# JuliaQuantumControl/QuOptimalControl.jl

Measured on AMD Instinct MI355X. Metric: GRAPE gradient-evals/sec, higher is better.
Workload: dtype f64; 1 GPU; C3: UnitaryGate 4x4, K=4, N=500 slices, ensemble E=1024 (one GPU, 1024 members/GPU), T=2.0; step = host->host grape_eval; parallelism=single GPU

## Files before the change

### quoptimalcontrol.jl_amd/csrc/cmatp.hpp

```cpp
#pragma once
#include <hip/hip_runtime.h>

#include "cmat.hpp"

namespace grape {

template <int N>
struct PMat {
    static constexpr int NC = N / 2;
    double re[N * (N / 2)];
    double im[N * (N / 2)];
};

GRAPE_DEV double pair_swap(double v)
{
    int lo = __double2loint(v), hi = __double2hiint(v);
    lo = __builtin_amdgcn_update_dpp(0, lo, 0xB1, 0xF, 0xF, true);
    hi = __builtin_amdgcn_update_dpp(0, hi, 0xB1, 0xF, 0xF, true);
    return __hiloint2double(hi, lo);
}

template <int N>
GRAPE_DEV void fetch_partner(PMat<N> &out, const PMat<N> &in)
{
// ... 222 lines not shown
                }
            }
            c.re[r + jl * N] = sr;
            c.im[r + jl * N] = si;
        }
        {
            double d = 0.0;
#pragma unroll
            for (int s = 0; s < N; ++s) {
                d = fma(g.re[s + jl * N], g.re[s + jl * N], d);
                d = fma(g.im[s + jl * N], g.im[s + jl * N], d);
            }
            c.re[jl + jl * N] = -d;
            c.im[jl + jl * N] = 0.0;
        }
#pragma unroll
        for (int rl = 0; rl < jl; ++rl) {
            double sr = 0.0, si = 0.0;
#pragma unroll
            for (int s = 0; s < N; ++s) {
                const double ar = g.re[s + rl * N], ai = -g.im[s + rl * N];
                const double br = g.re[s + jl * N], bi = g.im[s + jl * N];
                sr = fma(ar, br, sr); sr = fma(-ai, bi, sr);
                si = fma(ar, bi, si); si = fma(ai, br, si);
            }
            c.re[rl + jl * N] = -sr;
            c.im[rl + jl * N] = -si;
            c.re[jl + rl * N] = -sr;
            c.im[jl + rl * N] = si;
        }
    }
}

template <int N>
struct PAntiH {
    static constexpr int NC = N / 2;
    double di[NC];
    double ur[NC * NC], ui[NC * NC];
    double ore[NC * NC], oim[NC * NC];
};

template <int N>
GRAPE_DEV void pah_from_mat(PAntiH<N> &h, const PMat<N> &m)
{
    constexpr int NC = N / 2;
#pragma unroll
    for (int jl = 0; jl < NC; ++jl)
#pragma unroll
        for (int rl = 0; rl < NC; ++rl) {
            if (rl == jl)
                h.di[jl] = m.im[jl + jl * N];
            if (rl < jl) {
                h.ur[rl + jl * NC] = m.re[rl + jl * N];
                h.ui[rl + jl * NC] = m.im[rl + jl * N];
            }
            h.ore[rl + jl * NC] = m.re[NC + rl + jl * N];
            h.oim[rl + jl * NC] = m.im[NC + rl + jl * N];
        }
}

template <int N>
GRAPE_DEV void pah_of_scaled(PAntiH<N> &h, const PMat<N> &c, double zr, double zi)
{
    constexpr int NC = N / 2, NE = N * NC;
    PMat<N> Z;
#pragma unroll
    for (int e = 0; e < NE; ++e) {
        Z.re[e] = fma(c.re[e], zr, -c.im[e] * zi);
        Z.im[e] = fma(c.re[e], zi, c.im[e] * zr);
    }
#pragma unroll
    for (int jl = 0; jl < NC; ++jl)
#pragma unroll
        for (int rl = 0; rl < NC; ++rl) {
            if (rl == jl)
                h.di[jl] = Z.im[jl + jl * N];
            if (rl < jl) {
                h.ur[rl + jl * NC] = 0.5 * (Z.re[rl + jl * N] - Z.re[jl + rl * N]);
                h.ui[rl + jl * NC] = 0.5 * (Z.im[rl + jl * N] + Z.im[jl + rl * N]);
            }
            h.ore[rl + jl * NC] = 0.5 * (Z.re[NC + rl + jl * N] - pair_swap(Z.re[NC + jl + rl * N]));
            h.oim[rl + jl * NC] = 0.5 * (Z.im[NC + rl + jl * N] + pair_swap(Z.im[NC + jl + rl * N]));
        }
}

template <int N>
GRAPE_DEV void pah_own(PMat<N> &a, const PAntiH<N> &h)
{
    constexpr int NC = N / 2;
#pragma unroll
    for (int jl = 0; jl < NC; ++jl)
#pragma unroll
        for (int rl = 0; rl < NC; ++rl) {
            if (rl == jl) {
                a.re[rl + jl * N] = 0.0;
                a.im[rl + jl * N] = h.di[jl];
            } else if (rl < jl) {
                a.re[rl + jl * N] = h.ur[rl + jl * NC];
                a.im[rl + jl * N] = h.ui[rl + jl * NC];
            } else {
                a.re[rl + jl * N] = -h.ur[jl + rl * NC];
                a.im[rl + jl * N] = h.ui[jl + rl * NC];
            }
            a.re[NC + rl + jl * N] = h.ore[rl + jl * NC];
            a.im[NC + rl + jl * N] = h.oim[rl + jl * NC];
        }
}

template <int N>
GRAPE_DEV void pah_partner(PMat<N> &par, const PAntiH<N> &h)
{
    constexpr int NC = N / 2;
#pragma unroll
    for (int jl = 0; jl < NC; ++jl)
#pragma unroll
        for (int rl = 0; rl < NC; ++rl) {
            if (rl == jl) {
                par.re[rl + jl * N] = 0.0;
                par.im[rl + jl * N] = pair_swap(h.di[jl]);
            } else if (rl < jl) {
                const double vr = pair_swap(h.ur[rl + jl * NC]), vi = pair_swap(h.ui[rl + jl * NC]);
                par.re[rl + jl * N] = vr;
                par.im[rl + jl * N] = vi;
                par.re[jl + rl * N] = -vr;
                par.im[jl + rl * N] = vi;
            }
            par.re[NC + rl + jl * N] = -h.ore[jl + rl * NC];
            par.im[NC + rl + jl * N] = h.oim[jl + rl * NC];
        }
}

template <int N>
GRAPE_DEV void pmul_antih_a(PMat<N> &c, const PMat<N> &a, const PMat<N> &apar, const PMat<N> &b)
{
    constexpr int NC = N / 2;
#pragma unroll
    for (int jl = 0; jl < NC; ++jl)
#pragma unroll
        for (int r = 0; r < N; ++r) {
            double sr = 0.0, si = 0.0;
#pragma unroll
            for (int kl = 0; kl < NC; ++kl) {
                {
                    const double ar = a.re[r + kl * N], ai = a.im[r + kl * N];
                    const double br = b.re[kl + jl * N], bi = b.im[kl + jl * N];
                    if (r != kl) sr = fma(ar, br, sr);
                    sr = fma(-ai, bi, sr);
                    if (r != kl) si = fma(ar, bi, si);
                    si = fma(ai, br, si);
                }
                {
                    const int rb = flip_block<N>(r);
                    const double ar = apar.re[rb + kl * N], ai = apar.im[rb + kl * N];
                    const double br = b.re[NC + kl + jl * N], bi = b.im[NC + kl + jl * N];
                    if (rb != kl) sr = fma(ar, br, sr);
                    sr = fma(-ai, bi, sr);
                    if (rb != kl) si = fma(ar, bi, si);
                    si = fma(ai, br, si);
                }
            }
            c.re[r + jl * N] = sr;
            c.im[r + jl * N] = si;
        }
}

template <int N>
// ... 104 lines not shown
```

### quoptimalcontrol.jl_amd/csrc/sweep_pair.hip

```cpp
#include "cmatp.hpp"
#include "grape_kernels.hpp"

#ifndef GRAPE_ABL
#define GRAPE_ABL 0
#endif
#ifndef GRAPE_PD
#define GRAPE_PD 2
#endif
#ifndef GRAPE_PLAYOUT
#define GRAPE_PLAYOUT 0
#endif
#ifndef GRAPE_PD_EARLY
#define GRAPE_PD_EARLY 2
#endif
#ifndef GRAPE_PD_EARLY_AT
#define GRAPE_PD_EARLY_AT 0
#endif
#ifndef GRAPE_MBAR
#define GRAPE_MBAR 2
#endif

namespace grape {

enum { PMODE_GENERAL = 0, PMODE_GENERAL_KEEPL = 1, PMODE_UNITARY = 2, PMODE_UNITARY_AH = 3 };
// ... 13 lines not shown
{
#pragma unroll
    for (int jl = 0; jl < N / 2; ++jl)
#pragma unroll
        for (int r = 0; r < N; ++r)
            base[(size_t)gelem<N>(q, r, jl) * stride] = make_double2(m.re[r + jl * N], m.im[r + jl * N]);
}

template <int N>
GRAPE_DEV void pstore_ws_split(double2 *__restrict__ sbase, const unsigned (&voff)[2], size_t stride, const PMat<N> &m)
{
#pragma unroll
    for (int jl = 0; jl < N / 2; ++jl)
#pragma unroll
        for (int r = 0; r < N; ++r) {
            char *row = reinterpret_cast<char *>(sbase + (size_t)((r % (N / 2)) + jl * N) * stride);
            *reinterpret_cast<double2 *>(row + voff[r / (N / 2)]) = make_double2(m.re[r + jl * N], m.im[r + jl * N]);
        }
}

template <int N>
GRAPE_DEV void pload_ws(PMat<N> &m, const double2 *__restrict__ base, size_t stride, int q)
{
#pragma unroll
    for (int jl = 0; jl < N / 2; ++jl)
#pragma unroll
        for (int r = 0; r < N; ++r) {
            const double2 v = base[(size_t)gelem<N>(q, r, jl) * stride];
            m.re[r + jl * N] = v.x;
            m.im[r + jl * N] = v.y;
        }
}

template <int N>
GRAPE_DEV void pload_lds(PMat<N> &m, const double2 *s)
{
#pragma unroll
    for (int e = 0; e < N * (N / 2); ++e) {
        const double2 v = s[e];
        m.re[e] = v.x;
        m.im[e] = v.y;
    }
}

template <int N>
GRAPE_DEV void pstore_lds(double2 *s, const PMat<N> &m)
{
#pragma unroll
    for (int e = 0; e < N * (N / 2); ++e)
        s[e] = make_double2(m.re[e], m.im[e]);
}

GRAPE_DEV void pstamp(unsigned long long *__restrict__ st, int slot)
{
    if (st) {
        const unsigned long long t = __builtin_readcyclecounter();
        if ((threadIdx.x & 63) == 0)
            st[slot] = t;
    }
}

typedef double d2v __attribute__((ext_vector_type(2)));
struct PBuf {
    d2v v[8];
};

GRAPE_DEV void pbuf_issue(PBuf &b, unsigned voff0, unsigned voff1, const double2 *sb0, const double2 *sb1, const double2 *sb4,
                          const double2 *sb5)
{
    asm volatile("global_load_dwordx4 %0, %8, %10\n\t"
                 "global_load_dwordx4 %1, %8, %11\n\t"
                 "global_load_dwordx4 %2, %9, %10\n\t"
                 "global_load_dwordx4 %3, %9, %11\n\t"
                 "global_load_dwordx4 %4, %8, %12\n\t"
                 "global_load_dwordx4 %5, %8, %13\n\t"
                 "global_load_dwordx4 %6, %9, %12\n\t"
                 "global_load_dwordx4 %7, %9, %13"
                 : "=&v"(b.v[0]), "=&v"(b.v[1]), "=&v"(b.v[2]), "=&v"(b.v[3]), "=&v"(b.v[4]), "=&v"(b.v[5]), "=&v"(b.v[6]),
                   "=&v"(b.v[7])
                 : "v"(voff0), "v"(voff1), "s"(sb0), "s"(sb1), "s"(sb4), "s"(sb5)
                 : "memory");
}

template <int YOUNGER>
GRAPE_DEV void pbuf_wait(PBuf &b)
{
    asm volatile("s_waitcnt vmcnt(%8)"
                 : "+v"(b.v[0]), "+v"(b.v[1]), "+v"(b.v[2]), "+v"(b.v[3]), "+v"(b.v[4]), "+v"(b.v[5]), "+v"(b.v[6]), "+v"(b.v[7])
                 : "n"(YOUNGER)
                 : "memory");
}

GRAPE_DEV void pbuf_to_mat(PMat<4> &m, const PBuf &b)
{
#pragma unroll
    for (int e = 0; e < 8; ++e) {
        m.re[e] = b.v[e][0];
        m.im[e] = b.v[e][1];
    }
}

GRAPE_DEV void member_barrier(unsigned *cnt, unsigned target)
{
    asm volatile("s_waitcnt lgkmcnt(0)" ::: "memory");
    if ((threadIdx.x & 63) == 0)
        __hip_atomic_fetch_add(cnt, 1u, __ATOMIC_RELAXED, __HIP_MEMORY_SCOPE_WORKGROUP);
    while (__hip_atomic_load(cnt, __ATOMIC_RELAXED, __HIP_MEMORY_SCOPE_WORKGROUP) < target)
        __builtin_amdgcn_s_sleep(1);
    asm volatile("" ::: "memory");
}

GRAPE_DEV void lds_barrier()
{
    asm volatile("s_waitcnt lgkmcnt(0)" ::: "memory");
    __builtin_amdgcn_s_barrier();
    asm volatile("" ::: "memory");
}

template <int N, int SAND>
GRAPE_DEV double pfigure_of_merit(double zr, double zi)
{
    if (SAND) {
        const double inv = 1.0 / (double)N;
        const double ar = zr * inv, ai = zi * inv;
        return 1.0 - (ar * ar + ai * ai);
    }
    return zr * zr - zi * zi;
}

template <int N, int SAND>
GRAPE_DEV void pwrite_gradient(double *out, const double2 *s_bt, int K, const PMat<N> &M, double zr, double zi,
                               double gs, int p)
{
    constexpr int NE = N * (N / 2);
    PMat<N> Z;
#pragma unroll
    for (int e = 0; e < NE; ++e) {
        if (SAND) {
            Z.re[e] = M.re[e];
            Z.im[e] = M.im[e];
        } else {
            Z.re[e] = fma(M.re[e], zr, -M.im[e] * zi);
            Z.im[e] = fma(M.re[e], zi, M.im[e] * zr);
        }
    }
    double2 b0[NE], b1[NE];
#pragma unroll
    for (int e = 0; e < NE; ++e)
        b0[e] = s_bt[e];
    for (int c = 0; c < K; c += 2) {
        if (c + 1 < K) {
#pragma unroll
            for (int e = 0; e < NE; ++e)
                b1[e] = s_bt[(c + 1) * NE + e];
        }
        double re = 0.0;
#pragma unroll
        for (int e = 0; e < NE; ++e) {
            re = fma(b0[e].x, Z.re[e], re);
            re = fma(-b0[e].y, Z.im[e], re);
        }
        re += pair_swap(re);
        if (p == 0)
            out[c] = gs * re;
        if (c + 1 < K) {
            if (c + 2 < K) {
#pragma unroll
                for (int e = 0; e < NE; ++e)
                    b0[e] = s_bt[(c + 2) * NE + e];
            }
            double r1 = 0.0;
#pragma unroll
            for (int e = 0; e < NE; ++e) {
// ... 279 lines not shown
                    G.re[e] = fma(b0[e].x, x0, G.re[e]);
                    G.im[e] = fma(b0[e].y, x0, G.im[e]);
                }
            }
#pragma unroll
            for (int e = 0; e < NE; ++e)
                b0[e] = sB[c2 * NE + e];
#pragma unroll
            for (int e = 0; e < NE; ++e) {
                G.re[e] = fma(b1[e].x, x1, G.re[e]);
                G.im[e] = fma(b1[e].y, x1, G.im[e]);
            }
        }
        if (p.variant == 0) {
#pragma unroll
            for (int e = 0; e < NE; ++e) {
                const double2 a = sA[e];
                G.re[e] += a.x;
                G.im[e] += a.y;
            }
        }
        return nb;
    };
    auto slice = [&](int j, PMat<N> &G, double nb, const PMat<N> &Qin, PMat<N> &Qout, bool first) {
        PMat<N> P, Ppar;
        __builtin_amdgcn_sched_barrier(0);
        if (GRAPE_ABL & 32) P = G; else
        pexpm_t8<N, UNI>(P, G, p.s_forced, nb);
        __builtin_amdgcn_sched_barrier(0);
        if (!(GRAPE_ABL & 2))
        pstore_ws_split(p_Pk + (size_t)j * pstep, p_voff, stride, P);
        if (UNI && XGLDS && p.plast_lds && j == S - 1) {
#pragma unroll
            for (int e = 0; e < NE; ++e)
                s_plast[e * blockDim.x + threadIdx.x] = make_double2(P.re[e], P.im[e]);
        }
        PMat<N> R;
        if (GRAPE_ABL & 4) { R = Qin; R.re[0] += P.re[1]; } else if (first) {
            R = P;
        } else {
            fetch_partner(Ppar, P);
            pmul(R, P, Ppar, Qin);
        }
        Qout = R;
        if (MODE == PMODE_GENERAL && !VEC)
            pstore_ws(Xw + (size_t)j * NN * stride, stride, Qout, par);
        __builtin_amdgcn_sched_barrier(0);
    };
    if (__all(t0 + S <= Nsl)) {
        PMat<N> G;
        pset_identity(Q);
        int j = 0;
        for (; j + 1 < S; j += 2) {
            double nb = build(j, G);
            slice(j, G, nb, Q, Q2, j == 0);
            nb = build(j + 1, G);
            slice(j + 1, G, nb, Q2, Q, false);
        }
        if (j < S) {
            const double nb = build(j, G);
            slice(j, G, nb, Q, Q2, j == 0);
            Q = Q2;
        }
    } else {
        PMat<N> G;
        pset_identity(Q);
        for (int j = 0; j < S; ++j) {
            if (t0 + j < Nsl) {
                const double nb = build(j, G);
                slice(j, G, nb, Q, Q2, j == 0);
                Q = Q2;
            }
        }
    }

    pstamp(st, 1);
#if GRAPE_PD == 2
    PBuf bA, bB;
    constexpr int PD_EARLY = (SAND && GRAPE_PD_EARLY > 1) ? 1 : GRAPE_PD_EARLY;
    auto pd_issue = [&](PBuf &b, int jj) {
        const double2 *s0 = p_Pk + (size_t)max(jj, 0) * pstep;
        pbuf_issue(b, p_voff[0], p_voff[1], s0, s0 + CH, s0 + 4 * CH, s0 + 5 * CH);
    };
    auto pd_early = [&]() {
        if constexpr (PDASM && PD_EARLY >= 1) {
            const int jm0 = (XGLDS && p.plast_lds) ? S - 2 : S - 1;
            pd_issue(bA, jm0);
            if (PD_EARLY >= 2)
                pd_issue(bB, jm0 - 1);
        }
    };
    if (W == 1 || GRAPE_PD_EARLY_AT == 0)
        pd_early();
#endif
    PMat<N> Xs, Le;
    PAntiH<N> Ah;
    double zr = 0.0, zi = 0.0;
    {
        PMat<N> inc = Q, oth, tmp, ipar;
        for (int d = 1; d < 32; d <<= 1) {
            pshfl_up(oth, inc, 2 * d);
            if (cw >= d) {
                fetch_partner(ipar, inc);
                pmul(tmp, inc, ipar, oth);
                inc = tmp;
            }
        }
        if (!UNI) {
            pshfl_up(oth, inc, 2);
            if (cw == 0)
                pset_identity(oth);
        }
        if (W > 1) {
            if (cw == 31)
                pstore_lds(&s_tot[0][wbase_tot + wave][par * NE], inc);
            if (GRAPE_MBAR == 1 && UNI)
                member_barrier(&s_cnt[mb], (unsigned)W);
            else if (GRAPE_MBAR == 2 && UNI)
                lds_barrier();
            else
                __syncthreads();
#if GRAPE_PD == 2
            if (GRAPE_PD_EARLY_AT == 1)
                pd_early();
#endif
            if (wave > 0) {
                PMat<N> pre, wt, wtp;
                pload_lds(pre, &s_tot[0][wbase_tot][par * NE]);
                for (int w = 1; w < wave; ++w) {
                    pload_lds(wt, &s_tot[0][wbase_tot + w][par * NE]);
                    pload_lds(wtp, &s_tot[0][wbase_tot + w][(1 - par) * NE]);
                    pmul(tmp, wt, wtp, pre);
                    pre = tmp;
                }
                if (UNI) {
                    fetch_partner(ipar, inc);
                    pmul(tmp, inc, ipar, pre);
                    inc = tmp;
                } else {
                    fetch_partner(ipar, oth);
                    pmul(tmp, oth, ipar, pre);
                    oth = tmp;
                }
            }
        }
        if (UNI) {
            if (ch == CH - 1)
                pstore_lds(&s_tot[1][wbase_tot][par * NE], inc);
            if (GRAPE_MBAR == 1)
                member_barrier(&s_cnt[mb], (unsigned)(W > 1 ? 2 * W : W));
            else if (GRAPE_MBAR == 2)
                lds_barrier();
            else
                __syncthreads();
            PMat<N> T, C0, xi_m, xi_o;
            pload_lds(T, &s_tot[1][wbase_tot][par * NE]);
            if (SAND) {
                PMat<N> Em, Ep;
                {
                    PMat<N> xt_m, xt_o;
                    pload_lds(xt_m, sXt);
                    pload_lds(xt_o, sXt_o);
                    pmul(tmp, xt_m, xt_o, T);
                }
                {
                    PMat<N> Tp;
                    pload_lds(Tp, &s_tot[1][wbase_tot][(1 - par) * NE]);
                    pmul_ah_b(Em, T, Tp, tmp);
                }
                pload_lds(xi_m, sXi);
                ptrace_ah_b(zr, zi, xi_m, Em);
                fetch_partner(Ep, Em);
                pload_lds(xi_o, sXi_o);
                pmul_a_bh(C0, xi_m, xi_o, Em, Ep);
                pmul_ah_b(tmp, Em, Ep, xi_m);
#pragma unroll
                for (int e = 0; e < NE; ++e) {
                    C0.re[e] -= tmp.re[e];
                    C0.im[e] -= tmp.im[e];
                }
            } else {
                pload_lds(xi_m, sXX);
                pload_lds(xi_o, sXX_o);
                pmul(C0, xi_m, xi_o, T);
            }
            if constexpr (AH) {
                double tr_r, tr_i;
                ptrace(tr_r, tr_i, C0);
                zr = tr_r;
                zi = -tr_i;
                PAntiH<N> a0;
                pah_of_scaled(a0, C0, zr, zi);
                pah_own(C0, a0);
            }
            fetch_partner(ipar, inc);
            pmul(tmp, inc, ipar, C0);
            PMat<N> tp;
            fetch_partner(tp, tmp);
            pmul_a_bh(Xs, tmp, tp, inc, ipar);
            if constexpr (AH)
                pah_from_mat(Ah, Xs);
        } else {
            PMat<N> xi_m;
            pload_lds(xi_m, sXi);
            fetch_partner(ipar, oth);
            if (SAND) {
                pmul(tmp, oth, ipar, xi_m);
                PMat<N> tp;
                fetch_partner(tp, tmp);
                pmul_a_bh(Xs, tmp, tp, oth, ipar);
            } else {
                pmul(Xs, oth, ipar, xi_m);
            }
        }
    }
    if (!UNI) {
        PMat<N> inc = Q, oth, tmp, opar;
        for (int d = 1; d < 32; d <<= 1) {
            pshfl_down(oth, inc, 2 * d);
            if (cw + d < 32) {
                fetch_partner(opar, oth);
                pmul(tmp, oth, opar, inc);
                inc = tmp;
            }
        }
        pshfl_down(oth, inc, 2);
        if (cw == 31)
            pset_identity(oth);
        if (W > 1) {
            if (cw == 0)
                pstore_lds(&s_tot[1][wbase_tot + wave][par * NE], inc);
            __syncthreads();
            if (wave + 1 < W) {
                PMat<N> post, wt, wtp;
                pload_lds(post, &s_tot[1][wbase_tot + wave + 1][par * NE]);
                for (int w = wave + 2; w < W; ++w) {
                    pload_lds(wt, &s_tot[1][wbase_tot + w][par * NE]);
                    pload_lds(wtp, &s_tot[1][wbase_tot + w][(1 - par) * NE]);
                    pmul(tmp, wt, wtp, post);
                    post = tmp;
                }
                PMat<N> pp;
                fetch_partner(pp, post);
                pmul(tmp, post, pp, oth);
                oth = tmp;
            }
        }
        PMat<N> xt_m;
        pload_lds(xt_m, sXt);
        fetch_partner(opar, oth);
        if (SAND) {
            pmul_ah_b(tmp, oth, opar, xt_m);
            PMat<N> tp;
            fetch_partner(tp, tmp);
            pmul(Le, tmp, tp, oth);
        } else {
            pmul_ah_b(Le, oth, opar, xt_m);
        }
    }

    const double gs = SAND ? -1.0 : (p.variant == 0 ? -2.0 : 2.0);

    if (UNI) {
        pstamp(st, 2);
        pstamp(st, 3);
        PMat<N> M = Xs, Mp, tmp, PA, PB, Pp;
        auto products_ah = [&](const PMat<N> &P) {
            if constexpr (AH) {
                fetch_partner(Pp, P);
                pah_own(M, Ah);
                pah_partner(Mp, Ah);
                pmul_antih_a(tmp, M, Mp, P);
                pmul_ah_b_antih(Ah, P, Pp, tmp);
            }
        };
        auto step = [&](int j, const PMat<N> &P) {
            const int t = t0 + j;
            if ((GRAPE_ABL & 64) && t < Nsl) {
#pragma unroll
                for (int e = 0; e < NE; ++e) {
                    M.re[e] += P.re[e];
                    M.im[e] += P.im[e];
                }
                double acc = 0.0;
#pragma unroll
                for (int e = 0; e < NE; ++e)
                    acc += M.re[e] + M.im[e];
                if (par == 0) xg[j * K] = acc;
            } else
            if constexpr (AH) {
                if (t < Nsl) {
                    products_ah(P);
                    pwrite_gradient_antih(xg + j * K, sBT, K, Ah, gs, par);
                    if (t == Nsl - 1 && par == 0)
                        s_F[mb] = pfigure_of_merit<N, SAND>(zr, zi);
                }
            } else
            if (t < Nsl) {
                fetch_partner(Pp, P);
                fetch_partner(Mp, M);
                pmul(tmp, M, Mp, P);
                pmul_ah_b(M, P, Pp, tmp);
                if (!SAND) {
                    double tr_r, tr_i;
                    ptrace(tr_r, tr_i, M);
                    zr = tr_r;
                    zi = -tr_i;
                }
                if (DUMPW) {
                    fetch_partner(Mp, M);
                    pmul_a_bh(tmp, M, Mp, P, Pp);
                    pstore_ws(Xw + (size_t)j * NN * stride, stride, tmp, par);
                    if (t == Nsl - 1 && par == 0) {
                        p.zphi[2 * (size_t)k] = zr;
                        p.zphi[2 * (size_t)k + 1] = -zi;
                    }
                }
                if (GRAPE_ABL & 16) { if (par == 0) xg[j * K] = M.re[0] + zr; } else
                pwrite_gradient<N, SAND>(xg + j * K, sBT, K, M, zr, zi, gs, par);
                if (t == Nsl - 1 && par == 0)
                    s_F[mb] = pfigure_of_merit<N, SAND>(zr, zi);
            }
        };
        if (XGLDS && p.plast_lds) {
#pragma unroll
            for (int e = 0; e < NE; ++e) {
                const double2 v = s_plast[e * blockDim.x + threadIdx.x];
                PA.re[e] = v.x;
                PA.im[e] = v.y;
            }
        } else if (!PDASM) {
            pload_ws(PA, Pw + (size_t)(S - 1) * pstep, stride, par);
        }
        int j = S - 1;
#if GRAPE_PD == 1
        static_assert(!AH, "the anti-Hermitian sweep is written for GRAPE_PD 0 and 2");
        auto products = [&](int jj, const PMat<N> &P) {
            if (t0 + jj < Nsl) {
                fetch_partner(Pp, P);
                fetch_partner(Mp, M);
                pmul(tmp, M, Mp, P);
                pmul_ah_b(M, P, Pp, tmp);
            }
        };
        auto gradient = [&](int jj) {
            const int t = t0 + jj;
            if (t < Nsl) {
                if (!SAND) {
                    double tr_r, tr_i;
                    ptrace(tr_r, tr_i, M);
                    zr = tr_r;
                    zi = -tr_i;
                }
                pwrite_gradient<N, SAND>(xg + jj * K, sBT, K, M, zr, zi, gs, par);
                if (t == Nsl - 1 && par == 0)
                    s_F[mb] = pfigure_of_merit<N, SAND>(zr, zi);
            }
        };
        if (DUMPW) {
            for (; j >= 0; --j) {
                if (j < S - 1 || !(XGLDS && p.plast_lds))
                    pload_ws(PA, Pw + (size_t)j * pstep, stride, par);
                step(j, PA);
            }
        } else {
            pload_ws(PB, Pw + (size_t)max(j - 1, 0) * NN * stride, stride, par);
            for (; j >= 1; j -= 2) {
                products(j, PA);
                pload_ws(PA, Pw + (size_t)max(j - 2, 0) * NN * stride, stride, par);
                gradient(j);
                products(j - 1, PB);
                pload_ws(PB, Pw + (size_t)max(j - 3, 0) * NN * stride, stride, par);
                gradient(j - 1);
            }
            if (j == 0) {
                products(0, PA);
                gradient(0);
            }
        }
#elif GRAPE_PD == 2
        if constexpr (PDASM) {
            auto products = [&](int jj, const PMat<N> &P) {
                if (t0 + jj < Nsl) {
                    if constexpr (AH) {
                        products_ah(P);
                    } else {
                        fetch_partner(Pp, P);
                        fetch_partner(Mp, M);
                        pmul(tmp, M, Mp, P);
                        pmul_ah_b(M, P, Pp, tmp);
                    }
                }
            };
            auto gradient = [&](int jj) {
                const int t = t0 + jj;
                if constexpr (AH) {
                    if (t < Nsl) {
                        pwrite_gradient_antih(xg + jj * K, sBT, K, Ah, gs, par);
                        if (t == Nsl - 1 && par == 0)
                            s_F[mb] = pfigure_of_merit<N, SAND>(zr, zi);
                    }
                } else
                if (t < Nsl) {
                    if (!SAND) {
                        double tr_r, tr_i;
                        ptrace(tr_r, tr_i, M);
                        zr = tr_r;
                        zi = -tr_i;
                    }
                    pwrite_gradient<N, SAND>(xg + jj * K, sBT, K, M, zr, zi, gs, par);
                    if (t == Nsl - 1 && par == 0)
                        s_F[mb] = pfigure_of_merit<N, SAND>(zr, zi);
                }
            };
            const bool plast = XGLDS && p.plast_lds;
            const int jm = plast ? S - 2 : S - 1;
            if (PD_EARLY >= 1) {
                pbuf_wait<0>(bA);
                if (PD_EARLY >= 2)
                    pbuf_wait<0>(bB);
            } else {
                asm volatile("s_waitcnt vmcnt(0)" ::: "memory");
                pd_issue(bA, jm);
            }
            if (PD_EARLY < 2)
                pd_issue(bB, jm - 1);
            if (plast) {
                products(j, PA);
                gradient(j);
            }
            for (j = jm; j >= 1; j -= 2) {
                pbuf_wait<8>(bA);
                pbuf_to_mat(PA, bA);
                products(j, PA);
                pd_issue(bA, j - 2);
                gradient(j);
                pbuf_wait<8>(bB);
                pbuf_to_mat(PB, bB);
                products(j - 1, PB);
                pd_issue(bB, j - 3);
                gradient(j - 1);
            }
            if (j == 0) {
                pbuf_wait<8>(bA);
                pbuf_to_mat(PA, bA);
                products(0, PA);
                gradient(0);
            }
            pbuf_wait<0>(bA);
            pbuf_wait<0>(bB);
        } else {
            for (; j >= 1; j -= 2) {
                pload_ws(PB, Pw + (size_t)(j - 1) * pstep, stride, par);
                step(j, PA);
                if (j >= 2)
                    pload_ws(PA, Pw + (size_t)(j - 2) * pstep, stride, par);
                step(j - 1, PB);
            }
            if (j == 0)
                step(0, PA);
        }
#else
        for (; j >= 1; j -= 2) {
            if (!(GRAPE_ABL & 8)) pload_ws(PB, Pw + (size_t)(j - 1) * pstep, stride, par);
            step(j, PA);
            if (j >= 2 && !(GRAPE_ABL & 8))
                pload_ws(PA, Pw + (size_t)(j - 2) * pstep, stride, par);
            step(j - 1, PB);
        }
        if (j == 0)
            step(0, PA);
#endif
    } else {
        pstamp(st, 2);
        if (KEEPL) {
            PMat<N> X = Xs, Po, Pp, Xp, tmp;
            for (int j = 0; j < S; ++j) {
                const int t = t0 + j;
                if (t < Nsl) {
                    pstore_ws(Xw + (size_t)j * NN * stride, stride, X, par);
                    if (j + 1 < S) {
                        pload_ws(Po, Pw + (size_t)j * pstep, stride, par);
                        pload_ws(Pp, Pw + (size_t)j * pstep, stride, 1 - par);
                        if (SAND) {
                            fetch_partner(Xp, X);
                            pmul_a_bh(tmp, X, Xp, Po, Pp);
                            pmul(X, Po, Pp, tmp);
                        } else {
                            pmul(tmp, Po, Pp, X);
                            X = tmp;
                        }
                    }
                }
            }
        }

        pstamp(st, 3);
        if constexpr (VEC) {
            static_assert(N == 4 && !SAND && MODE == PMODE_GENERAL, "the vector sweep serves left multiplication at n = 4");
            constexpr int SV = kVecSlices;
            double xr[SV + 1][2], xi_[SV + 1][2];
            {
                const double a2 = pair_swap(Xs.re[2]), b2 = pair_swap(Xs.im[2]), a3 = pair_swap(Xs.re[3]), b3 = pair_swap(Xs.im[3]);
                xr[0][0] = par ? a2 : Xs.re[0];
                xi_[0][0] = par ? b2 : Xs.im[0];
                xr[0][1] = par ? a3 : Xs.re[1];
                xi_[0][1] = par ? b3 : Xs.im[1];
            }
            double wr[2], wi[2];
            {
                const double a2 = pair_swap(Le.re[2]), b2 = pair_swap(Le.im[2]), a3 = pair_swap(Le.re[3]), b3 = pair_swap(Le.im[3]);
                wr[0] = par ? a2 : Le.re[0];
                wi[0] = par ? b2 : Le.im[0];
                wr[1] = par ? a3 : Le.re[1];
                wi[1] = par ? b3 : Le.im[1];
            }
            PMat<N> Pj;
#pragma unroll
            for (int j = 0; j < SV; ++j) {
                if (j < S && t0 + j < Nsl) {
                    pload_ws(Pj, Pw + (size_t)j * pstep, stride, par);
                    double yr[4], yi[4];
#pragma unroll
                    for (int r = 0; r < 4; ++r) {
                        yr[r] = Pj.re[r] * xr[j][0];
                        yr[r] = fma(-Pj.im[r], xi_[j][0], yr[r]);
                        yr[r] = fma(Pj.re[r + 4], xr[j][1], yr[r]);
                        yr[r] = fma(-Pj.im[r + 4], xi_[j][1], yr[r]);
                        yi[r] = Pj.re[r] * xi_[j][0];
                        yi[r] = fma(Pj.im[r], xr[j][0], yi[r]);
                        yi[r] = fma(Pj.re[r + 4], xi_[j][1], yi[r]);
                        yi[r] = fma(Pj.im[r + 4], xr[j][1], yi[r]);
                    }
                    xr[j + 1][0] = yr[0] + pair_swap(yr[2]);
                    xi_[j + 1][0] = yi[0] + pair_swap(yi[2]);
                    xr[j + 1][1] = yr[1] + pair_swap(yr[3]);
                    xi_[j + 1][1] = yi[1] + pair_swap(yi[3]);
                } else {
                    xr[j + 1][0] = xr[j][0];
                    xi_[j + 1][0] = xi_[j][0];
                    xr[j + 1][1] = xr[j][1];
                    xi_[j + 1][1] = xi_[j][1];
                }
            }
#pragma unroll
            for (int j = SV - 1; j >= 0; --j) {
                if (j < S && t0 + j < Nsl) {
                    const int t = t0 + j;
                    pload_ws(Pj, Pw + (size_t)j * pstep, stride, par);
                    double lr[4], li[4];
                    lr[0] = wr[0]; li[0] = wi[0]; lr[1] = wr[1]; li[1] = wi[1];
                    lr[2] = pair_swap(wr[0]); li[2] = pair_swap(wi[0]); lr[3] = pair_swap(wr[1]); li[3] = pair_swap(wi[1]);
#pragma unroll
                    for (int jl = 0; jl < 2; ++jl) {
// ... 23 lines not shown
                    for (int c = 0; c < K; ++c) {
                        const double2 *bc = sB + (size_t)c * NE;
                        double ar = 0.0, ai = 0.0;
#pragma unroll
                        for (int jl = 0; jl < 2; ++jl) {
                            double ur = 0.0, ui = 0.0;
#pragma unroll
                            for (int r = 0; r < 4; ++r) {
                                const double2 b = bc[r + 4 * jl];
                                ur = fma(lr[r], b.x, ur);
                                ur = fma(li[r], b.y, ur);
                                ui = fma(lr[r], b.y, ui);
                                ui = fma(-li[r], b.x, ui);
                            }
                            ar = fma(ur, xr[j][jl], ar);
                            ar = fma(-ui, xi_[j][jl], ar);
                            ai = fma(ur, xi_[j][jl], ai);
                            ai = fma(ui, xr[j][jl], ai);
                        }
                        ar += pair_swap(ar);
                        ai += pair_swap(ai);
                        if (par == 0)
                            xg[j * K + c] = gs * fma(zr_, ar, -zi_ * ai);
                    }
                    if (t == Nsl - 1 && par == 0)
                        s_F[mb] = pfigure_of_merit<N, SAND>(zr_, zi_);
                }
            }
        } else {
        PMat<N> Lc = Le, Po, Pp, X, Xp, M, tmp, Lp;
        for (int j = S - 1; j >= 0; --j) {
            const int t = t0 + j;
            if (t < Nsl) {
                pload_ws(Po, Pw + (size_t)j * pstep, stride, par);
                pload_ws(Pp, Pw + (size_t)j * pstep, stride, 1 - par);
                if (SAND) {
                    fetch_partner(Lp, Lc);
                    pmul(tmp, Lc, Lp, Po);
                    pmul_ah_b(Lc, Po, Pp, tmp);
                } else {
                    pmul_ah_b(tmp, Po, Pp, Lc);
                    Lc = tmp;
                }
                if (KEEPL) {
                    pload_ws(X, Xw + (size_t)j * NN * stride, stride, par);
                } else if (j > 0) {
                    PMat<N> Qo, Qp;
                    pload_ws(Qo, Xw + (size_t)(j - 1) * NN * stride, stride, par);
                    pload_ws(Qp, Xw + (size_t)(j - 1) * NN * stride, stride, 1 - par);
                    if (SAND) {
                        pmul(tmp, Qo, Qp, Xs);
                        PMat<N> tp;
                        fetch_partner(tp, tmp);
                        pmul_a_bh(X, tmp, tp, Qo, Qp);
                    } else {
                        pmul(X, Qo, Qp, Xs);
                    }
                } else {
                    X = Xs;
                }
                if (KEEPL)
                    pstore_ws(p.costates + wbase + (size_t)j * NN * stride, stride, Lc, par);
                double zr, zi;
                ptrace_ah_b(zr, zi, X, Lc);
                fetch_partner(Xp, X);
                fetch_partner(Lp, Lc);
                pmul_a_bh(M, X, Xp, Lc, Lp);
                if (SAND) {
                    pmul_ah_b(tmp, Lc, Lp, X);
#pragma unroll
                    for (int e = 0; e < NE; ++e) {
                        M.re[e] -= tmp.re[e];
                        M.im[e] -= tmp.im[e];
                    }
                }
                pwrite_gradient<N, SAND>(xg + j * K, sBT, K, M, zr, zi, gs, par);
                if (t == Nsl - 1 && par == 0)
                    s_F[mb] = pfigure_of_merit<N, SAND>(zr, zi);
            }
        }
        }
    }
    __syncthreads();
    const int KN = K * Nsl;
    if (p.member_out && valid) {
        for (int q = L; q < KN; q += LT)
            out[q] = s_xg[q + chunk_of(q)];
        if (L == 0)
            out[KN] = s_F[mb];
    }
    {
        const int nmem = min(p.MPB, p.E - bi * p.MPB);
        const double *__restrict__ wb = wts_all + (size_t)bi * p.MPB;
        double *__restrict__ bout = p.block_out + (size_t)blockIdx.x * (KN + 1);
        const int mstride = CH * (SK + 1);
        for (int q = threadIdx.x; q <= KN; q += blockDim.x) {
            const int off = q + chunk_of(q);
            double acc = 0.0;
            for (int m = 0; m < nmem; ++m) {
                const double v = (q < KN) ? s_xg_all[m * mstride + off] : s_F[m];
                acc = fma(v, wb[m], acc);
            }
            bout[q] = acc;
            if (p.direct_dst)
                p.direct_dst[q] = acc;
        }
    }
    if (p.direct_flag) {
        __threadfence_system();
        __syncthreads();
        if (threadIdx.x == 0)
            __hip_atomic_store(p.direct_flag, p.direct_seq, __ATOMIC_RELEASE, __HIP_MEMORY_SCOPE_SYSTEM);
    }
    pstamp(st, 4);
    if (st && lane == 0) {
        st[6] = __builtin_amdgcn_s_memrealtime();
        st[7] = ((unsigned long long)__builtin_amdgcn_s_getreg(20 | (31 << 11)) << 32) |
                (unsigned)__builtin_amdgcn_s_getreg(4 | (31 << 11));
    }
}

template <int N, int SAND, int MODE, int MAXT, bool XGLDS, bool DUMPW = false, bool VEC = false>
__global__ __launch_bounds__(MAXT) void sweep_pair_kernel(const double2 *__restrict__ ops_all,
                                                          const double *__restrict__ x_all,
                                                          const double *__restrict__ wts_all,
                                                          const SweepParams p)
{
    sweep_pair_body<N, SAND, MODE, MAXT, XGLDS, DUMPW, VEC, XGLDS>(ops_all, x_all, wts_all, p);
}

template <int N, int SAND, int MODE, int MAXT, bool XGLDS, bool DUMPW = false, bool VEC = false>
__global__ __launch_bounds__(MAXT) void sweep_pair_build_kernel(const double2 *__restrict__ ops_all,
                                                                const double *__restrict__ x_all,
                                                                const double *__restrict__ wts_all,
                                                                const SweepParams p)
{
    sweep_pair_body<N, SAND, MODE, MAXT, XGLDS, DUMPW, VEC, false>(ops_all, x_all, wts_all, p);
}

template <int N>
__global__ __launch_bounds__(64) void pair_image_kernel(const double2 *__restrict__ ops_all, double2 *__restrict__ img_all,
                                                        int K, int E)
{
    constexpr int NN = N * N, NC = N / 2, NE = N * NC;
    constexpr bool AH = (N == 4);
    const int kl = blockIdx.x, L = threadIdx.x, LT = blockDim.x;
    if (kl >= E)
        return;
    const int NM = 2 * K + 4, PS = pair_image_ps(N, K), REC = 2 * PS;
    const double2 *__restrict__ ops = ops_all + (size_t)kl * (K + 3) * NN;
    double2 *__restrict__ rec = img_all + (size_t)kl * pair_image_d2(N, K);
    auto ah_weight = [&](int q, int c, int sl) {
        const int P0 = q * NC, Q0 = (1 - q) * NC;
        int jj, ii;
        double wt = 1.0;
        if (sl < 2)       { jj = ii = P0 + sl; }
        else if (sl < 4)  { jj = P0 + 1; ii = P0; wt = 2.0; }
        else if (sl < 6)  { jj = P0; ii = Q0; }
        else if (sl < 8)  { jj = P0 + 1; ii = Q0 + 1; }
        else              { jj = P0 + 1; ii = Q0; wt = 2.0; }
        const double2 b1 = ops[(size_t)(1 + c) * NN + jj + ii * N], b2 = ops[(size_t)(1 + c) * NN + ii + jj * N];
        const double bsr = 0.5 * (b1.x - b2.x), bsi = 0.5 * (b1.y + b2.y);
        const double v = sl < 2 ? -bsi : ((sl & 1) ? -wt * bsi : wt * bsr);
        return v;
    };
    for (int idx = L; idx < REC; idx += LT) {
// ... 196 lines not shown
```

Measured before the change: 12520 gradient-evals/s.

## Compute first-slice gradient from scan-shifted anti-Hermitian X instead of backward sweep

In the unitary anti-Hermitian mode, the gradient for each chunk's first slice (j=0) is now produced right after the scan. The anti-Hermitian X of the previous lane is shuffled up, handed across waves through LDS at wave boundaries, and taken from the seed for lane 0. The backward sweep therefore stops at j=1, skipping one products/gradient step and one propagator load per chunk. Prefetch loads become conditional assembly so no load is issued for slice 0. The cost is extra shuffles, LDS traffic, an additional __syncthreads for cross-wave fix-up, and more branchy inline assembly.

```diff
diff --git a/quoptimalcontrol.jl_amd/csrc/cmatp.hpp b/quoptimalcontrol.jl_amd/csrc/cmatp.hpp
--- a/quoptimalcontrol.jl_amd/csrc/cmatp.hpp
+++ b/quoptimalcontrol.jl_amd/csrc/cmatp.hpp
@@ -328,6 +328,51 @@
             h.ore[rl + jl * NC] = 0.5 * (Z.re[NC + rl + jl * N] - pair_swap(Z.re[NC + jl + rl * N]));
             h.oim[rl + jl * NC] = 0.5 * (Z.im[NC + rl + jl * N] + pair_swap(Z.im[NC + jl + rl * N]));
         }
+}
+
+template <int N, class H, class F>
+GRAPE_DEV void pah_each(H &h, F &&f)
+{
+    constexpr int NC = N / 2;
+#pragma unroll
+    for (int jl = 0; jl < NC; ++jl)
+        f(h.di[jl]);
+#pragma unroll
+    for (int jl = 0; jl < NC; ++jl)
+#pragma unroll
+        for (int rl = 0; rl < jl; ++rl) {
+            f(h.ur[rl + jl * NC]);
+            f(h.ui[rl + jl * NC]);
+        }
+#pragma unroll
+    for (int e = 0; e < NC * NC; ++e) {
+        f(h.ore[e]);
+        f(h.oim[e]);
+    }
+}
+
+template <int N>
+GRAPE_DEV void pah_shfl_up(PAntiH<N> &dst, const PAntiH<N> &src, int delta_lanes)
+{
+    dst = src;
+    pah_each<N>(dst, [&](double &v) { v = __shfl_up(v, delta_lanes, 64); });
+}
+
+template <int N>
+constexpr int pah_doubles() { return (N / 2) + (N / 2) * (N / 2 - 1) + 2 * (N / 2) * (N / 2); }
+
+template <int N>
+GRAPE_DEV void pah_store_lds(double *s, const PAntiH<N> &h)
+{
+    int i = 0;
+    pah_each<N>(h, [&](const double &v) { s[i++] = v; });
+}
+
+template <int N>
+GRAPE_DEV void pah_load_lds(PAntiH<N> &h, const double *s)
+{
+    int i = 0;
+    pah_each<N>(h, [&](double &v) { v = s[i++]; });
 }
 
 template <int N>
diff --git a/quoptimalcontrol.jl_amd/csrc/sweep_pair.hip b/quoptimalcontrol.jl_amd/csrc/sweep_pair.hip
--- a/quoptimalcontrol.jl_amd/csrc/sweep_pair.hip
+++ b/quoptimalcontrol.jl_amd/csrc/sweep_pair.hip
@@ -119,6 +119,25 @@
                  : "memory");
 }
 
+GRAPE_DEV void pbuf_issue_from1(PBuf &b, int jj, unsigned voff0, unsigned voff1, const double2 *sb0, const double2 *sb1,
+                             const double2 *sb4, const double2 *sb5)
+{
+    asm volatile("s_cmp_lt_i32 %14, 1\n\t"
+                 "s_cbranch_scc1 .Lpbuf_skip%=\n\t"
+                 "global_load_dwordx4 %0, %8, %10\n\t"
+                 "global_load_dwordx4 %1, %8, %11\n\t"
+                 "global_load_dwordx4 %2, %9, %10\n\t"
+                 "global_load_dwordx4 %3, %9, %11\n\t"
+                 "global_load_dwordx4 %4, %8, %12\n\t"
+                 "global_load_dwordx4 %5, %8, %13\n\t"
+                 "global_load_dwordx4 %6, %9, %12\n\t"
+                 "global_load_dwordx4 %7, %9, %13\n"
+                 ".Lpbuf_skip%=:"
+                 : "+v"(b.v[0]), "+v"(b.v[1]), "+v"(b.v[2]), "+v"(b.v[3]), "+v"(b.v[4]), "+v"(b.v[5]), "+v"(b.v[6]), "+v"(b.v[7])
+                 : "v"(voff0), "v"(voff1), "s"(sb0), "s"(sb1), "s"(sb4), "s"(sb5), "s"(jj)
+                 : "memory", "scc");
+}
+
 template <int YOUNGER>
 GRAPE_DEV void pbuf_wait(PBuf &b)
 {
@@ -126,6 +145,20 @@
                  : "+v"(b.v[0]), "+v"(b.v[1]), "+v"(b.v[2]), "+v"(b.v[3]), "+v"(b.v[4]), "+v"(b.v[5]), "+v"(b.v[6]), "+v"(b.v[7])
                  : "n"(YOUNGER)
                  : "memory");
+}
+
+GRAPE_DEV void pbuf_wait_behind(PBuf &b, int jj)
+{
+    asm volatile("s_cmp_lt_i32 %8, 1\n\t"
+                 "s_cbranch_scc1 .Lpbuf_w0%=\n\t"
+                 "s_waitcnt vmcnt(8)\n\t"
+                 "s_branch .Lpbuf_w1%=\n"
+                 ".Lpbuf_w0%=:\n\t"
+                 "s_waitcnt vmcnt(0)\n"
+                 ".Lpbuf_w1%=:"
+                 : "+v"(b.v[0]), "+v"(b.v[1]), "+v"(b.v[2]), "+v"(b.v[3]), "+v"(b.v[4]), "+v"(b.v[5]), "+v"(b.v[6]), "+v"(b.v[7])
+                 : "s"(jj)
+                 : "memory", "scc");
 }
 
 GRAPE_DEV void pbuf_to_mat(PMat<4> &m, const PBuf &b)
@@ -571,12 +604,22 @@
         const double2 *s0 = p_Pk + (size_t)max(jj, 0) * pstep;
         pbuf_issue(b, p_voff[0], p_voff[1], s0, s0 + CH, s0 + 4 * CH, s0 + 5 * CH);
     };
+    auto pd_issue_from1 = [&](PBuf &b, int jj) {
+        const double2 *s0 = p_Pk + (size_t)max(jj, 0) * pstep;
+        pbuf_issue_from1(b, __builtin_amdgcn_readfirstlane(jj), p_voff[0], p_voff[1], s0, s0 + CH, s0 + 4 * CH, s0 + 5 * CH);
+    };
     auto pd_early = [&]() {
         if constexpr (PDASM && PD_EARLY >= 1) {
             const int jm0 = (XGLDS && p.plast_lds) ? S - 2 : S - 1;
-            pd_issue(bA, jm0);
-            if (PD_EARLY >= 2)
-                pd_issue(bB, jm0 - 1);
+            if constexpr (AH) {
+                pd_issue_from1(bA, jm0);
+                if (PD_EARLY >= 2)
+                    pd_issue_from1(bB, jm0 - 1);
+            } else {
+                pd_issue(bA, jm0);
+                if (PD_EARLY >= 2)
+                    pd_issue(bB, jm0 - 1);
+            }
         }
     };
     if (W == 1 || GRAPE_PD_EARLY_AT == 0)
@@ -585,6 +628,15 @@
     PMat<N> Xs, Le;
     PAntiH<N> Ah;
     double zr = 0.0, zi = 0.0;
+    auto grad_scale = [&]() { return SAND ? -1.0 : (p.variant == 0 ? -2.0 : 2.0); };
+    constexpr bool HAND = AH;
+    constexpr int JLO = HAND ? 1 : 0;
+    auto hand_lane = [&]() {
+        int tx = threadIdx.x;
+        asm volatile("" : "+v"(tx));
+        return tx - mb * LT;
+    };
+    auto hand_slot = [&](int w, int q) { return reinterpret_cast<double *>(&s_tot[0][wbase_tot + w][q * NE]); };
     {
         PMat<N> inc = Q, oth, tmp, ipar;
         for (int d = 1; d < 32; d <<= 1) {
@@ -680,6 +732,8 @@
                 zi = -tr_i;
                 PAntiH<N> a0;
                 pah_of_scaled(a0, C0, zr, zi);
+                if (const int hl = hand_lane(); hl < 2)
+                    pah_store_lds<N>(hand_slot(W - 1, hl), a0);
                 pah_own(C0, a0);
             }
             fetch_partner(ipar, inc);
@@ -687,8 +741,21 @@
             PMat<N> tp;
             fetch_partner(tp, tmp);
             pmul_a_bh(Xs, tmp, tp, inc, ipar);
-            if constexpr (AH)
+            if constexpr (AH) {
                 pah_from_mat(Ah, Xs);
+                const int hl = hand_lane(), hwave = __builtin_amdgcn_readfirstlane(hl >> 6), hcw = (hl & 63) >> 1, hpar = hl & 1;
+                if (hcw == 31 && hwave + 1 < W)
+                    pah_store_lds<N>(hand_slot(hwave, hpar), Ah);
+                PAntiH<N> Ain;
+                pah_shfl_up(Ain, Ah, 2);
+                if (hwave == 0 && hcw == 0)
+                    pah_load_lds<N>(Ain, hand_slot(W - 1, hpar));
+                if (t0 < Nsl && (hwave == 0 || hcw != 0)) {
+                    pwrite_gradient_antih(xg, sBT, K, Ain, grad_scale(), par);
+                    if (t0 == Nsl - 1 && par == 0)
+                        s_F[mb] = pfigure_of_merit<N, SAND>(zr, zi);
+                }
+            }
         } else {
             PMat<N> xi_m;
             pload_lds(xi_m, sXi);
@@ -748,7 +815,7 @@
         }
     }
 
-    const double gs = SAND ? -1.0 : (p.variant == 0 ? -2.0 : 2.0);
+    const double gs = grad_scale();
 
     if (UNI) {
         pstamp(st, 2);
@@ -818,7 +885,7 @@
                 PA.re[e] = v.x;
                 PA.im[e] = v.y;
             }
-        } else if (!PDASM) {
+        } else if (!PDASM && S - 1 >= JLO) {
             pload_ws(PA, Pw + (size_t)(S - 1) * pstep, stride, par);
         }
         int j = S - 1;
@@ -904,6 +971,40 @@
             };
             const bool plast = XGLDS && p.plast_lds;
             const int jm = plast ? S - 2 : S - 1;
+            if constexpr (HAND) {
+                if (PD_EARLY >= 1) {
+                    pbuf_wait<0>(bA);
+                    if (PD_EARLY >= 2)
+                        pbuf_wait<0>(bB);
+                } else {
+                    asm volatile("s_waitcnt vmcnt(0)" ::: "memory");
+                    pd_issue_from1(bA, jm);
+                }
+                if (PD_EARLY < 2)
+                    pd_issue_from1(bB, jm - 1);
+                if (plast) {
+                    products(j, PA);
+                    gradient(j);
+                }
+                for (j = jm; j >= 2; j -= 2) {
+                    pbuf_wait<8>(bA);
+                    pbuf_to_mat(PA, bA);
+                    products(j, PA);
+                    pd_issue_from1(bA, j - 2);
+                    gradient(j);
+                    pbuf_wait_behind(bB, __builtin_amdgcn_readfirstlane(j - 2));
+                    pbuf_to_mat(PB, bB);
+                    products(j - 1, PB);
+                    pd_issue_from1(bB, j - 3);
+                    gradient(j - 1);
+                }
+                pbuf_wait<0>(bA);
+                if (j == 1) {
+                    pbuf_to_mat(PA, bA);
+                    products(1, PA);
+                    gradient(1);
+                }
+            } else {
             if (PD_EARLY >= 1) {
                 pbuf_wait<0>(bA);
                 if (PD_EARLY >= 2)
@@ -938,27 +1039,28 @@
             }
             pbuf_wait<0>(bA);
             pbuf_wait<0>(bB);
+            }
         } else {
-            for (; j >= 1; j -= 2) {
+            for (; j >= JLO + 1; j -= 2) {
                 pload_ws(PB, Pw + (size_t)(j - 1) * pstep, stride, par);
                 step(j, PA);
-                if (j >= 2)
+                if (j >= JLO + 2)
                     pload_ws(PA, Pw + (size_t)(j - 2) * pstep, stride, par);
                 step(j - 1, PB);
             }
-            if (j == 0)
-                step(0, PA);
+            if (j == JLO)
+                step(JLO, PA);
         }
 #else
-        for (; j >= 1; j -= 2) {
+        for (; j >= JLO + 1; j -= 2) {
             if (!(GRAPE_ABL & 8)) pload_ws(PB, Pw + (size_t)(j - 1) * pstep, stride, par);
             step(j, PA);
-            if (j >= 2 && !(GRAPE_ABL & 8))
+            if (j >= JLO + 2 && !(GRAPE_ABL & 8))
                 pload_ws(PA, Pw + (size_t)(j - 2) * pstep, stride, par);
             step(j - 1, PB);
         }
-        if (j == 0)
-            step(0, PA);
+        if (j == JLO)
+            step(JLO, PA);
 #endif
     } else {
         pstamp(st, 2);
@@ -1148,6 +1250,19 @@
         }
     }
     __syncthreads();
+    if constexpr (HAND) {
+        if (W > 1) {
+            const int hl = hand_lane();
+            if (hl >= 64 && (hl & 62) == 0 && t0 < Nsl) {
+                PAntiH<N> Ain;
+                pah_load_lds<N>(Ain, hand_slot((hl >> 6) - 1, hl & 1));
+                pwrite_gradient_antih(xg, sBT, K, Ain, gs, par);
+                if (t0 == Nsl - 1 && par == 0)
+                    s_F[mb] = pfigure_of_merit<N, SAND>(zr, zi);
+            }
+            __syncthreads();
+        }
+    }
     const int KN = K * Nsl;
     if (p.member_out && valid) {
         for (int q = L; q < KN; q += LT)
```

Result: no change. 12670 gradient-evals/s, median of 6 (+1.2%).
